# rvignolo/RayTracing.jl

Measured on NVIDIA B200. Metric: segments/sec for segmentize!, higher is better.
Workload: dtype f64

## Files before the change

### raytracing.jl_b200/csrc/eval3.cuh

```cuda
#pragma once
#include "topo.cuh"

namespace rt {

#ifndef RT_EVAL3_THREADS
#define RT_EVAL3_THREADS 32
#endif
constexpr int kEval3Threads = RT_EVAL3_THREADS;
#ifndef RT_EVAL3_MIN_BLOCKS
#define RT_EVAL3_MIN_BLOCKS 32
#endif
#ifndef RT_EVAL3_ALIGN
#define RT_EVAL3_ALIGN 8
#endif
#ifndef RT_EVAL3_PF_AHEAD
#define RT_EVAL3_PF_AHEAD 64
#endif

__device__ __forceinline__ void prefetch_l2(const void *p) { asm volatile("prefetch.global.L2 [%0];" ::"l"(p)); }

__device__ __forceinline__ bool eval3_cross(const Line &trk, const Line &L, P2 &out, bool &redo) {
    const double a = trk.b * L.a, b = L.b * trk.a;
    const double fa = fabs(a), fb = fabs(b);
    const bool par = fabs(a - b) <= kRtol * (fa > fb ? fa : fb);
    const Recip rd = recip_prepare(a - b);
    bool ok = rd.ok;
    out.x = div_try<false>(trk.c * L.b - L.c * trk.b, rd, ok);
    out.y = div_try<false>(trk.a * L.c - L.a * trk.c, rd, ok);
    redo = !ok;
    return par;
}

__global__ void __launch_bounds__(kEval3Threads, RT_EVAL3_MIN_BLOCKS) k_eval3(const __grid_constant__ WalkParams P) {
    const unsigned FULL = 0xffffffffu;
    const DevMesh &m = P.m;
    const int lane = threadIdx.x & 31;
    const long long w = blockIdx.x * (long long)(kEval3Threads / 32) + (threadIdx.x >> 5);
    const long long slot = P.unit_begin + (w >> 5);
    if (slot >= P.unit_end) return;
    if (P.cancel && *P.cancel) return;
    const int ls = (int)(w & 31);
    const long long unit = P.ch.order ? P.ch.order[slot] : slot;
#if RT_EVAL3_PF_AHEAD > 0
    {
        const long long slot_a = slot + RT_EVAL3_PF_AHEAD;
        if (slot_a < P.unit_end) {
            const long long unit_a = P.ch.order ? P.ch.order[slot_a] : slot_a;
            const long long cidx_a = unit_a * 32 + ls;
            const char *recs = (const char *)(P.pool + (cidx_a - P.pool_slot_base) * kRecBlock);
            if (lane < 4) prefetch_l2(recs + 128 * lane);
            else if (lane == 4) prefetch_l2(P.ch.count + cidx_a);
            else if (lane == 5) prefetch_l2(P.ch.prefix + cidx_a);
            else if (lane == 6) prefetch_l2(P.ch.seed_qx + cidx_a);
            else if (lane == 7) prefetch_l2(P.ch.seed_qy + cidx_a);
        }
    }
#endif
    const long long cidx = unit * 32 + ls;
    const int pb0 = (int)(cidx - P.pool_slot_base);
    int pb = pb0;
    const int cnt = P.ch.count[cidx];
    const int rec_first = P.pool[(long long)pb * kRecBlock + lane];
    const int prefix = P.ch.prefix[cidx];
    const double seedx = P.ch.seed_qx[cidx], seedy = P.ch.seed_qy[cidx];
    const int blk = P.ch.unit_block[unit];
    const long long t = 32LL * blk + ls;
    if (t >= P.n_tracks || t < P.trk_begin || t >= P.trk_end) return;
    const int nch = P.ch.nch[t];
    const long long ubase = P.ch.unit_base[blk];
    const int az = P.t.azim[t];
    const Line trk{P.t.a[t], P.t.b[t], P.t.c[t]};
    const long long off_t = P.offsets[t];
    const int j = (int)(unit - ubase);
    if (j >= nch) return;
    if (cnt <= 0) return;
    int rec_cur = lane < cnt ? rec_first : 1;
    int rec_prev = 1;
    int rec;

    const unsigned long long pol_keep = l2_policy_keep();
    const bool right = P.ang.phi[az] < kPi / 2;
    const double delta = P.vol ? P.ang.delta_eff[az] : 0.0;
    const long long base = off_t - P.offset_base + prefix;
    double cqx = seedx, cqy = seedy;
    int cfast = j > 0;
    double lsum = 0.0;
    bool bad = false, any_lit = false;
    const int rot = (lane + 31) & 31;

    const int sh = (int)(base & (RT_EVAL3_ALIGN - 1));
    const int src_lane = (lane - sh) & 31;
    for (int i0 = 0; i0 < cnt + sh; i0 += 32) {
        const int v = i0 + lane - sh;
        int rec_next = 1;
        {
            const int i1 = i0 + 32;
            if (i1 < cnt && (i1 & (kRecBlock - 1)) == 0) pb = P.pool_next[pb];
            if (i1 + lane < cnt) rec_next = P.pool[(long long)pb * kRecBlock + ((i1 + lane) & (kRecBlock - 1))];
        }
        {
            const int a = __shfl_sync(FULL, rec_prev, src_lane), b = __shfl_sync(FULL, rec_cur, src_lane);
            rec = lane < sh ? a : b;
        }
        const bool fast = (rec & 1) == 0;
        const unsigned h = (unsigned)rec >> 2;
        const unsigned cell = fast ? h / 3u : h;
        const unsigned kin = h - 3u * cell;
        const bool exit1 = (rec & 2) != 0;
        P2 q{0.0, 0.0};
        bool par = false, redo = false;
        Line L{0.0, 0.0, 0.0};
        if (fast) {
            unsigned kout = kin + (exit1 ? 1u : 2u);
            kout = kout >= 3u ? kout - 3u : kout;
            double elen;
            ldg256_keep(m.edges + (3u * cell + kout), pol_keep, L.a, L.b, L.c, elen);
            par = eval3_cross(trk, L, q, redo);
        }
        if (redo) par = intersection(trk, L, q);
        const double rx = __shfl_sync(FULL, q.x, rot), ry = __shfl_sync(FULL, q.y, rot);
        const int rfast = __shfl_sync(FULL, (int)fast, rot);
        const bool from_left = lane != 0 && v != 0;
        P2 p{from_left ? rx : cqx, from_left ? ry : cqy};
        const bool have = (from_left ? rfast : cfast) != 0;
        cqx = rx;
        cqy = ry;
        cfast = rfast;
        if (fast && !have) {
            double elen;
            ldg256_keep(m.edges + (3u * cell + kin), pol_keep, L.a, L.b, L.c, elen);
            intersection(trk, L, p);
        }
        if (fast) {
            const double dx = p.x - q.x, dy = p.y - q.y;
            const double l = sqrt(dx * dx + dy * dy);
            const long long so = base + v;
            P.opx[so] = p.x;
            P.opy[so] = p.y;
            P.oqx[so] = q.x;
            P.oqy[so] = q.y;
            P.olen[so] = l;
            P.oelem[so] = (int)cell + 1;
            if (P.vol) atomicAdd(&P.vol[cell], delta * l);
            lsum += l;
            const bool kin_lt_kout = (kin == 0u) || (kin == 1u && exit1);
            const bool lt = right ? (p.x < q.x) : (p.x > q.x);
            const bool in_first = lt || (p.x == q.x && !kin_lt_kout);
            bad = bad || par || !in_first || !(l > P.lmin);
        } else if ((unsigned)v < (unsigned)cnt) {
            any_lit = true;
        }
        rec_prev = rec_cur;
        rec_cur = rec_next;
    }
    if (bad) atomicExch(P.verify_fail, 1);

    if (__any_sync(FULL, any_lit)) {
        pb = pb0;
        for (int i0 = 0; i0 < cnt; i0 += 32) {
            if (i0 && (i0 & (kRecBlock - 1)) == 0) pb = P.pool_next[pb];
            const int v = i0 + lane;
            const int r = v < cnt ? P.pool[(long long)pb * kRecBlock + (v & (kRecBlock - 1))] : 0;
            if (r & 1) {
                const int cell = r >> 2;
                P2 p, q;
                int e_p, e_q;
                intersections(m, cell, trk, right, p, q, e_p, e_q);
                const double l = norm2(p.x - q.x, p.y - q.y);
                const long long so = base + v;
                P.opx[so] = p.x;
                P.opy[so] = p.y;
                P.oqx[so] = q.x;
                P.oqy[so] = q.y;
                P.olen[so] = l;
                P.oelem[so] = cell + 1;
                if (P.vol) atomicAdd(&P.vol[cell], delta * l);
                lsum += l;
            }
        }
    }
    if (P.tsum) {
        for (int o = 16; o > 0; o >>= 1) lsum += __shfl_down_sync(FULL, lsum, o);
        if (lane == 0) atomicAdd(&P.tsum[t], lsum);
    }
}

}
```

### raytracing.jl_b200/csrc/rt_b200.cu

```cuda
#include "../../include/rt_b200.h"

#include <dlfcn.h>

#include <algorithm>
#include <cstdarg>
#include <cstdio>
#include <cstring>
#include <string>
#include <vector>

#include "scan.cuh"
#include "sweep.cuh"
#include "eval3.cuh"
#include "march.cuh"
#include "topo.cuh"
#include "trace.cuh"

using namespace rt;

typedef struct ncclComm *ncclComm_t;
typedef struct {
    char internal[128];
} ncclUniqueId;
typedef int ncclResult_t;
// ... 55 lines not shown
    cudaEvent_t ev_aux = nullptr;
    bool area_valid = false;
    long long *h_pin = nullptr;
    DevBuf b_cell_bin;
    DevBuf b_scratch, b_gcounts, b_gcursor;
    DevBuf b_tsum;
    DevBuf b_pool, b_pool_next, b_pool_cursor;
    int count_batches = 0;
    unsigned long long trace_gen = 0;
    struct PlanKey {
        unsigned long long gen = ~0ULL;
        double chunk_len = -1.0;
        int band = -1, order_grid = -1;
        double band_min = -1.0, band_div = -1.0;
        long long n = -1;
        bool operator==(const PlanKey &o) const { return gen == o.gen && chunk_len == o.chunk_len && band == o.band && order_grid == o.order_grid && n == o.n &&
                   band_min == o.band_min && band_div == o.band_div; }
    } plan_key;
    bool plan_has_order = false;
    int opt_debug_clear_pool = 0;
    double opt_band_cost = 28.0;
    int opt_plan_cache = 1;
    int opt_optimistic = 1;
    bool skip_optimistic_once = false;
    int optimistic_cancels = 0;
    unsigned long long fit_gen = ~0ULL;

    int opt_band_chunks = 1;
    double opt_band_min = 0.0625;
    double opt_band_div = 8.0;
    long long opt_pool_slots = 0;
    double opt_pool_extra = 1.25;
    int opt_pipeline = 3;
    int verify_fallbacks = 0;
    int opt_debug_verify_fail = 0;
    double tau_ms = 0.0;
    cudaEvent_t ev2[2] = {nullptr, nullptr};
    int opt_order_grid = 32;
    const int *order_eval = nullptr;
    int opt_order_classes = 3;
    int n_sm = 148;
    long long n_units = 0;
    double opt_chunk_segments = 208.0;
    double opt_target_walkers = 148.0 * 2048.0 * 4.0;
    double sum_len = 0.0;
    double edge_sum = 0.0, area = 0.0;
    long long total_segments = 0;
    long long cap_cfg = 0;
    long long cap = 0;
    DevBuf b_seg_d, b_seg_e;
    double *s_px = nullptr, *s_py = nullptr, *s_qx = nullptr, *s_qy = nullptr, *s_len = nullptr;
    int *s_elem = nullptr;
    long long res_trk_begin = 0, res_trk_end = 0, res_off_base = 0, res_nseg = 0;
    bool vol_valid = false;

    double phase_ms[6] = {0, 0, 0, 0, 0, 0};
    double stats[8] = {0, 0, 0, 0, 0, 0, 0, 0};

    NcclApi nccl;
    ncclComm_t comm = nullptr;
    int n_ranks = 1, rank = 0;
    cudaStream_t coll_stream = nullptr;
    DevBuf b_vol_alt;
    int vol_cur = 0;
    double *vol_acc = nullptr;
    cudaEvent_t ev_fill_done = nullptr;
    cudaEvent_t ev_vol_free[2] = {nullptr, nullptr};
    bool ev_vol_used[2] = {false, false};
    bool voln_done = false;
    int voln_ready = -1;
};

static inline unsigned long long *d_counters(rt_ctx *c) { return (unsigned long long *)c->b_ctrl.p; }
static inline unsigned long long *d_bad(rt_ctx *c) { return (unsigned long long *)c->b_ctrl.p + 4; }
static inline int *d_verify(rt_ctx *c) { return (int *)((unsigned long long *)c->b_ctrl.p + 5); }
static inline int *d_guard(rt_ctx *c) { return (int *)((unsigned long long *)c->b_ctrl.p + 5) + 1; }
constexpr int kPinWords = 32, kPinCtrlInit = 16, kPinCtrl = 24;

static int fail(rt_ctx *c, int code, const char *fmt, ...) {
    char buf[512];
    va_list ap;
    va_start(ap, fmt);
    vsnprintf(buf, sizeof(buf), fmt, ap);
    va_end(ap);
    if (c) c->err = buf;
    return code;
}

#define CK(call)                                                                                              \
    do {                                                                                                      \
        cudaError_t e_ = (call);                                                                              \
        if (e_ != cudaSuccess)                                                                                \
            return fail(ctx, RT_ERR_CUDA, "%s failed at %s:%d: %s", #call, __FILE__, __LINE__,              \
                        cudaGetErrorString(e_));                                                              \
    } while (0)

static cudaError_t ensure(DevBuf &b, size_t bytes) {
    if (bytes <= b.bytes && b.p) return cudaSuccess;
    if (b.p) cudaFree(b.p);
    b.p = nullptr;
    b.bytes = 0;
    cudaError_t e = cudaMalloc(&b.p, bytes ? bytes : 1);
    if (e == cudaSuccess) b.bytes = bytes;
    return e;
}
static void release(DevBuf &b) {
    if (b.p) cudaFree(b.p);
    b.p = nullptr;
    b.bytes = 0;
}

static inline unsigned blocks_for(long long n, int threads) { return (unsigned)((n + threads - 1) / threads); }

template <typename Tin, typename Tout>
static cudaError_t exclusive_scan(rt_ctx *ctx, const Tin *in, Tout *out, long long n, Tout carry = Tout(0), ScanGuard guard = ScanGuard{}) {
    long long n_tiles = (n + kScanTile - 1) / kScanTile;
    cudaError_t e = ensure(ctx->b_tile, sizeof(Tout) * (size_t)n_tiles);
    if (e != cudaSuccess) return e;
    Tout *tiles = (Tout *)ctx->b_tile.p;
    k_scan_tile_sums<Tin, Tout><<<(unsigned)n_tiles, kScanThreads, 0, ctx->stream>>>(in, tiles, n);
    k_scan_tile_offsets<Tout><<<1, kScanThreads, 0, ctx->stream>>>(tiles, n_tiles);
    k_scan_apply<Tin, Tout><<<(unsigned)n_tiles, kScanThreads, 0, ctx->stream>>>(in, out, tiles, n, carry, guard);
    return cudaGetLastError();
}

extern "C" const char *rt_version(void) { return "rt_b200 0.1 (sm_100a, fp64, fmad=false)"; }

extern "C" int rt_create(rt_ctx **out, int device) {
    if (!out) return RT_ERR_ARG;
    *out = nullptr;
    int n = 0;
    cudaError_t e = cudaGetDeviceCount(&n);
    if (e != cudaSuccess || n <= 0 || device < 0 || device >= n) return RT_ERR_CUDA;
    rt_ctx *ctx = new rt_ctx();
    ctx->device = device;
    cudaDeviceGetAttribute(&ctx->n_sm, cudaDevAttrMultiProcessorCount, device);
    if (ctx->n_sm <= 0) ctx->n_sm = 148;
    if (cudaSetDevice(device) != cudaSuccess || cudaStreamCreateWithFlags(&ctx->stream, cudaStreamNonBlocking) != cudaSuccess ||
        cudaEventCreate(&ctx->tev[0]) != cudaSuccess || cudaEventCreate(&ctx->tev[1]) != cudaSuccess ||
        cudaEventCreate(&ctx->ev2[0]) != cudaSuccess || cudaEventCreate(&ctx->ev2[1]) != cudaSuccess) {
        delete ctx;
        return RT_ERR_CUDA;
    }
    if (cudaHostAlloc((void **)&ctx->h_pin, kPinWords * sizeof(long long), cudaHostAllocDefault) != cudaSuccess) {
        delete ctx;
        return RT_ERR_NOMEM;
    }
    for (int ph = 0; ph < 6; ++ph)
        for (int q = 0; q < 2; ++q)
            if (cudaEventCreate(&ctx->pev[ph][q]) != cudaSuccess) {
                delete ctx;
                return RT_ERR_CUDA;
            }
    *out = ctx;
    return RT_OK;
}

extern "C" void rt_destroy(rt_ctx *ctx) {
    if (!ctx) return;
    cudaSetDevice(ctx->device);
    if (ctx->coll_stream) cudaStreamSynchronize(ctx->coll_stream);
    if (ctx->stream) cudaStreamSynchronize(ctx->stream);
    if (ctx->comm && ctx->nccl.CommDestroy) ctx->nccl.CommDestroy(ctx->comm);
    DevBuf *all[] = {&ctx->b_cell_ptrs, &ctx->b_xy,      &ctx->b_cell_nodes, &ctx->b_nc_ptrs,  &ctx->b_nc_data, &ctx->b_nbr,     &ctx->b_cells,
                     &ctx->b_edges,   &ctx->b_qual,       &ctx->b_bdist,    &ctx->b_sc,      &ctx->b_grid_ptrs, &ctx->b_grid_nodes,
                     &ctx->b_ang_d,   &ctx->b_ang_i,      &ctx->b_trk_d,    &ctx->b_trk_i,   &ctx->b_trk_l,   &ctx->b_trk_c,
                     &ctx->b_err,     &ctx->b_count,      &ctx->b_status,   &ctx->b_offsets, &ctx->b_tile,    &ctx->b_vol,
                     &ctx->b_voln,    &ctx->b_ctrl,       &ctx->b_seg_d,   &ctx->b_seg_e,
                     &ctx->b_twin,    &ctx->b_he,         &ctx->b_node_reach,
                     &ctx->b_nch,     &ctx->b_blk_chunks, &ctx->b_unit_base, &ctx->b_unit_block, &ctx->b_ch_i, &ctx->b_ch_d,
                     &ctx->b_order,   &ctx->b_okeys,      &ctx->b_ohist,     &ctx->b_tsum,
                     &ctx->b_scratch, &ctx->b_gcounts,   &ctx->b_gcursor,   &ctx->b_cell_bin,
                     &ctx->b_omega,   &ctx->b_sigma,     &ctx->b_tau,
                     &ctx->b_pool,    &ctx->b_pool_next, &ctx->b_pool_cursor,
                     &ctx->b_area,    &ctx->b_factor,    &ctx->b_layout,    &ctx->b_vol_alt,  &ctx->b_exc};
    for (DevBuf *b : all) release(*b);
    for (int ph = 0; ph < 6; ++ph)
        for (int q = 0; q < 2; ++q)
            if (ctx->pev[ph][q]) cudaEventDestroy(ctx->pev[ph][q]);
    if (ctx->coll_stream) {
        cudaStreamSynchronize(ctx->coll_stream);
        cudaStreamDestroy(ctx->coll_stream);
    }
    for (cudaEvent_t e : {ctx->ev_fill_done, ctx->ev_vol_free[0], ctx->ev_vol_free[1]})
        if (e) cudaEventDestroy(e);
    if (ctx->aux_stream) cudaStreamDestroy(ctx->aux_stream);
    if (ctx->ev_aux) cudaEventDestroy(ctx->ev_aux);
    if (ctx->stream) cudaStreamDestroy(ctx->stream);
    if (ctx->h_pin) cudaFreeHost(ctx->h_pin);
    delete ctx;
}

extern "C" const char *rt_last_error(const rt_ctx *ctx) { return ctx ? ctx->err.c_str() : "null context"; }

extern "C" int rt_host_alloc(void **ptr, size_t bytes) {
    return cudaHostAlloc(ptr, bytes ? bytes : 1, cudaHostAllocDefault) == cudaSuccess ? RT_OK : RT_ERR_NOMEM;
}
extern "C" int rt_host_free(void *ptr) { return cudaFreeHost(ptr) == cudaSuccess ? RT_OK : RT_ERR_CUDA; }

static void tic(rt_ctx *ctx, int ph) { cudaEventRecord(ctx->pev[ph][0], ctx->stream); }
static void toc(rt_ctx *ctx, int ph) {
    cudaEventRecord(ctx->pev[ph][1], ctx->stream);
    ctx->pev_dirty[ph] = true;
}
static void collect_phase_ms(rt_ctx *ctx) {
    for (int ph = 0; ph < 6; ++ph) {
        if (!ctx->pev_dirty[ph]) continue;
        float ms = 0.f;
        if (cudaEventSynchronize(ctx->pev[ph][1]) == cudaSuccess && cudaEventElapsedTime(&ms, ctx->pev[ph][0], ctx->pev[ph][1]) == cudaSuccess)
            ctx->phase_ms[ph] = (double)ms;
        ctx->pev_dirty[ph] = false;
    }
}

extern "C" int rt_mesh_upload(rt_ctx *ctx, int32_t n_nodes, const double *xy, int32_t n_cells, const int32_t *cell_ptrs,
                              const int32_t *cell_data, const int32_t *node_cell_ptrs, const int32_t *node_cell_data,
                              const double bb_min[2], const double bb_max[2]) {
    if (!ctx) return RT_ERR_ARG;
    if (n_nodes < 3 || n_cells < 1 || !xy || !cell_ptrs || !cell_data || (!node_cell_ptrs != !node_cell_data) || (!bb_min != !bb_max))
        return fail(ctx, RT_ERR_ARG, "rt_mesh_upload: null or empty mesh arrays");
    const bool dev_nc = node_cell_ptrs == nullptr;
    const bool dev_bb = bb_min == nullptr;
    bool mixed = false;
    for (int32_t c = 0; c < n_cells; ++c) {
        const int nn = cell_ptrs[c + 1] - cell_ptrs[c];
        if (nn == 4)
            mixed = true;
        else if (nn != 3)
            return fail(ctx, RT_ERR_ARG, "rt_mesh_upload: cell %d has %d nodes (triangles and quadrilaterals only)", c + 1, nn);
    }
    if (mixed && dev_nc) return fail(ctx, RT_ERR_ARG, "rt_mesh_upload: a mesh with quadrilaterals needs the vertex -> cells table from the caller");
    const size_t n_cd = (size_t)(cell_ptrs[n_cells] - 1);
    CK(cudaSetDevice(ctx->device));
    cudaStream_t st = ctx->stream;
    tic(ctx, 0);
    size_t n_nc = dev_nc ? (size_t)3 * n_cells : (size_t)(node_cell_ptrs[n_nodes] - 1);
    CK(ensure(ctx->b_xy, sizeof(double2) * (size_t)n_nodes));
    CK(ensure(ctx->b_cell_nodes, sizeof(int) * n_cd));
    CK(ensure(ctx->b_nc_ptrs, sizeof(int) * ((size_t)n_nodes + 1)));
    CK(ensure(ctx->b_nc_data, sizeof(int) * n_nc));
    CK(ensure(ctx->b_nbr, sizeof(int) * 3 * (size_t)n_cells));
    CK(ensure(ctx->b_cells, sizeof(CellRec) * (size_t)n_cells));
    CK(ensure(ctx->b_edges, sizeof(EdgeRec) * 3 * (size_t)n_cells));
    CK(ensure(ctx->b_qual, sizeof(float) * (size_t)n_cells));
    CK(ensure(ctx->b_bdist, sizeof(float) * (size_t)n_cells));
    CK(ensure(ctx->b_sc, sizeof(MeshScalars)));
    const size_t tab_n[3] = {n_cd, dev_nc ? 0 : (size_t)n_nodes + 1, dev_nc ? 0 : n_nc};
    CK(ensure(ctx->b_scratch, sizeof(int32_t) * (tab_n[0] + tab_n[1] + tab_n[2])));
    CK(cudaMemcpyAsync(ctx->b_xy.p, xy, sizeof(double) * 2 * (size_t)n_nodes, cudaMemcpyHostToDevice, st));
    const int32_t *tab_src[3] = {cell_data, node_cell_ptrs, node_cell_data};
    void *tab_dst[3] = {ctx->b_cell_nodes.p, ctx->b_nc_ptrs.p, ctx->b_nc_data.p};
    size_t tab_off = 0;
    for (int q = 0; q < 3; ++q) {
        if (tab_n[q] == 0) continue;
        int32_t *stage = (int32_t *)ctx->b_scratch.p + tab_off;
        CK(cudaMemcpyAsync(stage, tab_src[q], sizeof(int32_t) * tab_n[q], cudaMemcpyHostToDevice, st));
        k_to_zero_based<<<blocks_for((long long)tab_n[q], 256), 256, 0, st>>>(stage, (int *)tab_dst[q], (long long)tab_n[q]);
        tab_off += tab_n[q];
    }

    if (mixed) {
        DevBuf stage;
        CK(ensure(stage, sizeof(int32_t) * ((size_t)n_cells + 1)));
        CK(ensure(ctx->b_cell_ptrs, sizeof(int) * ((size_t)n_cells + 1)));
        CK(cudaMemcpyAsync(stage.p, cell_ptrs, sizeof(int32_t) * ((size_t)n_cells + 1), cudaMemcpyHostToDevice, st));
        k_to_zero_based<<<blocks_for((long long)n_cells + 1, 256), 256, 0, st>>>((const int32_t *)stage.p, (int *)ctx->b_cell_ptrs.p, (long long)n_cells + 1);
        CK(cudaStreamSynchronize(st));
        release(stage);
    }
    if (dev_nc) {
        DevBuf deg, cur;
        CK(ensure(deg, sizeof(int) * (size_t)n_nodes));
        CK(ensure(cur, sizeof(int) * (size_t)n_nodes));
        CK(cudaMemsetAsync(deg.p, 0, sizeof(int) * (size_t)n_nodes, st));
        CK(cudaMemsetAsync(cur.p, 0, sizeof(int) * (size_t)n_nodes, st));
        k_nc_count<<<blocks_for(3LL * n_cells, 256), 256, 0, st>>>(n_cells, (const int *)ctx->b_cell_nodes.p, (int *)deg.p);
        CK((exclusive_scan<int, int>(ctx, (const int *)deg.p, (int *)ctx->b_nc_ptrs.p, (long long)n_nodes)));
        k_nc_fill<<<blocks_for(3LL * n_cells, 256), 256, 0, st>>>(n_cells, (const int *)ctx->b_cell_nodes.p, (const int *)ctx->b_nc_ptrs.p,
                                                                   (int *)cur.p, (int *)ctx->b_nc_data.p);
        k_nc_sort<<<blocks_for(n_nodes, 256), 256, 0, st>>>(n_nodes, (const int *)ctx->b_nc_ptrs.p, (int *)ctx->b_nc_data.p);
        CK(cudaGetLastError());
        CK(cudaStreamSynchronize(st));
        release(deg);
        release(cur);
    }
    double bbv[4];
    if (dev_bb) {
        DevBuf dbb;
        CK(ensure(dbb, sizeof(double) * 4));
        const double init[4] = {INFINITY, INFINITY, -INFINITY, -INFINITY};
        CK(cudaMemcpyAsync(dbb.p, init, sizeof(init), cudaMemcpyHostToDevice, st));
        k_bbox<<<std::min(1024u, blocks_for(n_nodes, 256)), 256, 0, st>>>((const double2 *)ctx->b_xy.p, n_nodes, (double *)dbb.p);
        CK(cudaMemcpyAsync(bbv, dbb.p, sizeof(bbv), cudaMemcpyDeviceToHost, st));
        CK(cudaStreamSynchronize(st));
        release(dbb);
        bb_min = bbv;
        bb_max = bbv + 2;
    }
    DevMesh &m = ctx->m;
    m.n_nodes = n_nodes;
    m.n_cells = n_cells;
    m.xy = (const double2 *)ctx->b_xy.p;
    m.cell_nodes = (const int *)ctx->b_cell_nodes.p;
    m.cell_ptrs = mixed ? (const int *)ctx->b_cell_ptrs.p : nullptr;
    m.nc_ptrs = (const int *)ctx->b_nc_ptrs.p;
    m.nc_data = (const int *)ctx->b_nc_data.p;
// ... 1304 lines not shown
    if (r != 0) return fail(ctx, RT_ERR_NCCL, "ncclCommInitRank: %s", ctx->nccl.GetErrorString ? ctx->nccl.GetErrorString(r) : "?");
    if (!ctx->coll_stream) {
        if (cudaStreamCreateWithFlags(&ctx->coll_stream, cudaStreamNonBlocking) != cudaSuccess ||
            cudaEventCreateWithFlags(&ctx->ev_fill_done, cudaEventDisableTiming) != cudaSuccess ||
            cudaEventCreateWithFlags(&ctx->ev_vol_free[0], cudaEventDisableTiming) != cudaSuccess ||
            cudaEventCreateWithFlags(&ctx->ev_vol_free[1], cudaEventDisableTiming) != cudaSuccess)
            return fail(ctx, RT_ERR_CUDA, "rt_comm_init: cannot create the collective stream");
    }
    ctx->n_ranks = n_ranks;
    ctx->rank = rank;
    return RT_OK;
}

extern "C" int rt_volumes(rt_ctx *ctx, double *volumes) {
    if (!ctx) return RT_ERR_ARG;
    const bool have = ctx->segmented && ctx->vol_valid;
    const bool coll = ctx->comm && ctx->coll_stream;
    if (!have && !(coll && ctx->has_mesh)) return fail(ctx, RT_ERR_ARG, "rt_volumes: run rt_segmentize with volumes enabled first");
    CK(cudaSetDevice(ctx->device));
    cudaStream_t st = ctx->stream;
    int nc = ctx->m.n_cells;
    CK(ensure(ctx->b_voln, sizeof(double) * ((size_t)nc + 1)));
    const double *src = ctx->vol_acc ? ctx->vol_acc : (const double *)ctx->b_vol.p;
    if (!have) {
        CK(cudaStreamSynchronize(ctx->coll_stream));
        CK(ensure(ctx->b_vol, sizeof(double) * ((size_t)nc + 1)));
        CK(cudaMemsetAsync(ctx->b_vol.p, 0, sizeof(double) * ((size_t)nc + 1), st));
        const double one = 1.0;
        CK(cudaMemcpyAsync((double *)ctx->b_vol.p + nc, &one, sizeof(double), cudaMemcpyHostToDevice, st));
        CK(cudaStreamSynchronize(st));
        src = (const double *)ctx->b_vol.p;
    }
    if (coll) {
        cudaStream_t cs = ctx->coll_stream;
        CK(cudaEventRecord(ctx->ev_fill_done, st));
        CK(cudaStreamWaitEvent(cs, ctx->ev_fill_done, 0));
        CK(cudaEventRecord(ctx->pev[5][0], cs));
        ncclResult_t r = ctx->nccl.AllReduce(src, ctx->b_voln.p, (size_t)nc + 1, ncclFloat64, ncclSum, ctx->comm, cs);
        if (r != 0) return fail(ctx, RT_ERR_NCCL, "ncclAllReduce: %s", ctx->nccl.GetErrorString ? ctx->nccl.GetErrorString(r) : "?");
        k_normalise<<<blocks_for(nc, 256), 256, 0, cs>>>((const double *)ctx->b_voln.p, (double *)ctx->b_voln.p, nc, (double)ctx->n2);
        CK(cudaGetLastError());
        CK(cudaEventRecord(ctx->pev[5][1], cs));
        ctx->pev_dirty[5] = true;
        if (have) {
            CK(cudaEventRecord(ctx->ev_vol_free[ctx->vol_cur], cs));
            ctx->ev_vol_used[ctx->vol_cur] = true;
            ctx->voln_ready = ctx->vol_cur;
        }
        if (volumes || !have) CK(cudaStreamSynchronize(cs));
        if (!have) return fail(ctx, RT_ERR_ARG, "rt_volumes: this rank's rt_segmentize failed; it joined the all-reduce with a zero contribution and the failed-rank flag");
    } else {
        if (!ctx->voln_done) {
            tic(ctx, 5);
            k_normalise<<<blocks_for(nc, 256), 256, 0, st>>>(src, (double *)ctx->b_voln.p, nc, (double)ctx->n2);
            CK(cudaGetLastError());
            toc(ctx, 5);
        }
        ctx->voln_ready = -1;
        if (volumes) CK(cudaStreamSynchronize(st));
    }
    if (volumes) {
        CK(cudaMemcpy(volumes, ctx->b_voln.p, sizeof(double) * (size_t)nc, cudaMemcpyDeviceToHost));
        if (coll) {
            double failed = 0.0;
            CK(cudaMemcpy(&failed, (const double *)ctx->b_voln.p + nc, sizeof(double), cudaMemcpyDeviceToHost));
            if (failed != 0.0)
                return fail(ctx, RT_ERR_PEER, "rt_volumes: rt_segmentize failed on %d rank(s) of the communicator: the volumes miss their tracks", (int)failed);
        }
    }
    return RT_OK;
}


__device__ __forceinline__ unsigned long long splitmix64(unsigned long long &x) {
    unsigned long long z = (x += 0x9e3779b97f4a7c15ull);
    z = (z ^ (z >> 30)) * 0xbf58476d1ce4e5b9ull;
    z = (z ^ (z >> 27)) * 0x94d049bb133111ebull;
    return z ^ (z >> 31);
}

__global__ void k_selftest_division(long long n, unsigned long long seed, int exp_span, unsigned long long *mismatch) {
    long long i = blockIdx.x * (long long)blockDim.x + threadIdx.x;
    if (i >= n) return;
    unsigned long long st = seed + 0x632be59bd9b4e019ull * (unsigned long long)(i + 1);
    unsigned long long bad = 0;
    for (int rep = 0; rep < 64; ++rep) {
        unsigned long long r1 = splitmix64(st), r2 = splitmix64(st), r3 = splitmix64(st);
        int e1 = 1023 + (int)(r3 % (2 * exp_span + 1)) - exp_span, e2 = 1023 + (int)((r3 >> 20) % (2 * exp_span + 1)) - exp_span;
        e1 = min(max(e1, 0), 2046);
        e2 = min(max(e2, 1), 2046);
        unsigned long long mx = r1 & 0xfffffffffffffull, mn = r2 & 0xfffffffffffffull;
        int kind = (int)((r3 >> 44) & 15);
        if (kind == 1) mx = 0;
        if (kind == 2) mx = 0xfffffffffffffull;
        if (kind == 3) mn = 0xfffffffffffffull;
        if (kind == 4) mn = 0;
        double x = __longlong_as_double((long long)(((r1 >> 63) << 63) | ((unsigned long long)e1 << 52) | mx));
        double d = __longlong_as_double((long long)(((r2 >> 63) << 63) | ((unsigned long long)e2 << 52) | mn));
        if (kind == 5) x = 0.0;
        if (kind == 6) x = -0.0;
        Recip r = recip_prepare(d);
        double q1 = div_shared(x, r), q2 = x / d;
        if (__double_as_longlong(q1) != __double_as_longlong(q2)) bad++;
    }
    if (bad) atomicAdd(mismatch, bad);
}

extern "C" int rt_selftest_division(rt_ctx *ctx, int64_t n_threads, uint64_t seed, int32_t exp_span, int64_t *mismatches) {
    if (!ctx || !mismatches || n_threads < 1 || exp_span < 0 || exp_span > 1022) return RT_ERR_ARG;
    CK(cudaSetDevice(ctx->device));
    DevBuf d;
    CK(ensure(d, sizeof(unsigned long long)));
    CK(cudaMemsetAsync(d.p, 0, sizeof(unsigned long long), ctx->stream));
    k_selftest_division<<<blocks_for(n_threads, 256), 256, 0, ctx->stream>>>(n_threads, seed, exp_span, (unsigned long long *)d.p);
    CK(cudaGetLastError());
    unsigned long long h = 0;
    CK(cudaMemcpyAsync(&h, d.p, sizeof(h), cudaMemcpyDeviceToHost, ctx->stream));
    CK(cudaStreamSynchronize(ctx->stream));
    release(d);
    *mismatches = (int64_t)h;
    return RT_OK;
}

extern "C" int rt_stats(rt_ctx *ctx, double stats[8]) {
    if (!ctx || !stats) return RT_ERR_ARG;
    cudaSetDevice(ctx->device);
    collect_phase_ms(ctx);
    ctx->stats[5] = ctx->phase_ms[2];
    ctx->stats[6] = ctx->phase_ms[4];
    ctx->stats[7] = ctx->phase_ms[3];
    memcpy(stats, ctx->stats, sizeof(ctx->stats));
    return RT_OK;
}

extern "C" int rt_info(rt_ctx *ctx, const char *key, double *value) {
    if (!ctx || !key || !value) return RT_ERR_ARG;
    std::string k(key);
    if (k == "verify_fallbacks")
        *value = ctx->verify_fallbacks;
    else if (k == "tau_ms")
        *value = ctx->tau_ms;
    else if (k == "n_units")
        *value = (double)ctx->n_units;
    else if (k == "segment_capacity")
        *value = (double)ctx->cap;
    else if (k == "rho")
        *value = ctx->area > 0.0 ? ctx->edge_sum / (kPi * ctx->area) : 0.0;
    else if (k == "band_cost")
        *value = ctx->opt_band_cost;
    else if (k == "count_batches")
        *value = (double)ctx->count_batches;
    else if (k == "optimistic_cancels")
        *value = (double)ctx->optimistic_cancels;
    else
        return fail(ctx, RT_ERR_ARG, "rt_info: unknown key %s", key);
    return RT_OK;
}

extern "C" int rt_debug_chunk_stats(rt_ctx *ctx, double out[8]) {
    if (!ctx || !out || !ctx->segmented || ctx->n_units <= 0) return fail(ctx, RT_ERR_ARG, "rt_debug_chunk_stats: call rt_segmentize first");
    CK(cudaSetDevice(ctx->device));
    CK(cudaStreamSynchronize(ctx->stream));
    const long long n = ctx->n_shard, n_units = ctx->n_units, n_blocks = (n + 31) / 32;
    const size_t nc = (size_t)n_units * 32;
    std::vector<int> nch((size_t)n), ublk((size_t)n_units), seed(nc), cnt(nc);
    std::vector<long long> ubase((size_t)n_blocks + 1);
    CK(cudaMemcpy(nch.data(), ctx->b_nch.p, sizeof(int) * nch.size(), cudaMemcpyDeviceToHost));
    CK(cudaMemcpy(ublk.data(), ctx->b_unit_block.p, sizeof(int) * ublk.size(), cudaMemcpyDeviceToHost));
    CK(cudaMemcpy(ubase.data(), ctx->b_unit_base.p, sizeof(long long) * ubase.size(), cudaMemcpyDeviceToHost));
    CK(cudaMemcpy(seed.data(), ctx->b_ch_i.p, sizeof(int) * nc, cudaMemcpyDeviceToHost));
    CK(cudaMemcpy(cnt.data(), (const int *)ctx->b_ch_i.p + 2 * nc, sizeof(int) * nc, cudaMemcpyDeviceToHost));
    double work = 0, voids = 0, sum = 0, mx = 0;
    for (long long u = 0; u < n_units; ++u) {
        const long long b = ublk[(size_t)u];
        const int j = (int)(u - ubase[(size_t)b]);
        for (int l = 0; l < 32; ++l) {
            const long long t = 32 * b + l;
            if (t >= n || j >= nch[(size_t)t]) continue;
            const size_t c = (size_t)u * 32 + l;
            if (j >= 1 && seed[c] < 0) voids += 1;
            if (cnt[c] > 0) {
                work += 1;
                sum += cnt[c];
                mx = std::max(mx, (double)cnt[c]);
            }
        }
    }
    const double mean = work > 0 ? sum / work : 0.0;
    double over15 = 0, over2 = 0;
    for (long long u = 0; u < n_units; ++u) {
        const long long b = ublk[(size_t)u];
        const int j = (int)(u - ubase[(size_t)b]);
        double umax = 0, usum = 0;
        for (int l = 0; l < 32; ++l) {
            const long long t = 32 * b + l;
            if (t >= n || j >= nch[(size_t)t]) continue;
            const double c = (double)std::max(cnt[(size_t)u * 32 + l], 0);
            umax = std::max(umax, c);
            usum += c;
        }
        over15 += umax;
        over2 += usum / 32.0;
    }
    out[0] = work;
    out[1] = voids;
    out[2] = mean;
    out[3] = mx;
    out[4] = over15;
    out[5] = over2;
    out[6] = (double)nc;
    out[7] = (double)n_units;
    return RT_OK;
}

extern "C" int rt_phase_ms(rt_ctx *ctx, double ms[6]) {
    if (!ctx || !ms) return RT_ERR_ARG;
    cudaSetDevice(ctx->device);
    collect_phase_ms(ctx);
    memcpy(ms, ctx->phase_ms, sizeof(ctx->phase_ms));
    return RT_OK;
}

extern "C" int rt_timer_start(rt_ctx *ctx) {
    if (!ctx) return RT_ERR_ARG;
    CK(cudaSetDevice(ctx->device));
    if (ctx->coll_stream) CK(cudaStreamSynchronize(ctx->coll_stream));
    CK(cudaStreamSynchronize(ctx->stream));
    CK(cudaEventRecord(ctx->tev[0], ctx->stream));
    return RT_OK;
}

extern "C" int rt_timer_stop(rt_ctx *ctx, double *elapsed_ms) {
    if (!ctx || !elapsed_ms) return RT_ERR_ARG;
    if (ctx->voln_ready >= 0) CK(cudaStreamWaitEvent(ctx->stream, ctx->ev_vol_free[ctx->voln_ready], 0));
    CK(cudaEventRecord(ctx->tev[1], ctx->stream));
    CK(cudaEventSynchronize(ctx->tev[1]));
    float ms = 0.f;
    CK(cudaEventElapsedTime(&ms, ctx->tev[0], ctx->tev[1]));
    *elapsed_ms = (double)ms;
    return RT_OK;
}

extern "C" int rt_set_option(rt_ctx *ctx, const char *name, double value) {
    if (!ctx || !name) return RT_ERR_ARG;
    std::string n(name);
    if (n == "chunk_segments" && value >= 1.0)
        ctx->opt_chunk_segments = value;
    else if (n == "target_walkers" && value >= 1.0)
        ctx->opt_target_walkers = value;
    else if (n == "order_grid" && value >= 0.0 && value <= 256.0)
        ctx->opt_order_grid = (int)value;
    else if (n == "pipeline" && (value == 0.0 || value == 1.0 || value == 3.0))
        ctx->opt_pipeline = (int)value;
    else if (n == "debug_clear_pool")
        ctx->opt_debug_clear_pool = value != 0.0;
    else if (n == "band_cost" && value >= 0.0)
        ctx->opt_band_cost = value;
    else if (n == "order_classes" && value >= 0.0 && value <= 64.0)
        ctx->opt_order_classes = (int)value;
    else if (n == "plan_cache")
        ctx->opt_plan_cache = value != 0.0;
    else if (n == "optimistic")
        ctx->opt_optimistic = value != 0.0;
    else if (n == "band_chunks")
        ctx->opt_band_chunks = value != 0.0;
    else if (n == "band_min" && value >= 0.0)
        ctx->opt_band_min = value;
    else if (n == "band_div" && value >= 1.0 && value <= 64.0)
        ctx->opt_band_div = value;
    else if (n == "pool_slots" && value >= 0.0)
        ctx->opt_pool_slots = (long long)value;
    else if (n == "pool_extra" && value >= 0.0)
        ctx->opt_pool_extra = value;
    else if (n == "debug_verify_fail")
        ctx->opt_debug_verify_fail = value != 0.0;
    else
        return fail(ctx, RT_ERR_ARG, "rt_set_option: unknown option or bad value: %s", name);
    return RT_OK;
}
```

Measured before the change: 32.91 billion.

## Stage segment outputs in shared-memory ring and flush with bulk async copies

Replaces the per-lane scattered global stores of segment columns with writes into a per-warp shared-memory ring. Full windows are then flushed to global memory by TMA bulk copies (cp.async.bulk) issued by lane 0, and unaligned edge elements are stored directly. This removes the old alignment-shift shuffle path and aims to produce fully coalesced, asynchronous output writes. In exchange it adds about 6KB of shared memory per one-warp block, which may cut occupancy, and adds proxy fences and wait_group synchronisation.

```diff
diff --git a/raytracing.jl_b200/csrc/eval3.cuh b/raytracing.jl_b200/csrc/eval3.cuh
--- a/raytracing.jl_b200/csrc/eval3.cuh
+++ b/raytracing.jl_b200/csrc/eval3.cuh
@@ -10,14 +10,34 @@
 #ifndef RT_EVAL3_MIN_BLOCKS
 #define RT_EVAL3_MIN_BLOCKS 32
 #endif
-#ifndef RT_EVAL3_ALIGN
-#define RT_EVAL3_ALIGN 8
-#endif
+#ifndef RT_EVAL3_WIN
+#define RT_EVAL3_WIN 64
+#endif
+#ifndef RT_EVAL3_FLUSH
+#define RT_EVAL3_FLUSH 1
+#endif
+constexpr int kEval3Win = RT_EVAL3_WIN;
+constexpr int kEval3Ring = 2 * kEval3Win;
 #ifndef RT_EVAL3_PF_AHEAD
 #define RT_EVAL3_PF_AHEAD 64
 #endif
 
 __device__ __forceinline__ void prefetch_l2(const void *p) { asm volatile("prefetch.global.L2 [%0];" ::"l"(p)); }
+
+__device__ __forceinline__ void bulk_s2g(void *dst, const void *src, int bytes) {
+    asm volatile("cp.async.bulk.global.shared::cta.bulk_group [%0], [%1], %2;" ::"l"(dst), "r"((unsigned)__cvta_generic_to_shared(src)),
+                 "r"(bytes)
+                 : "memory");
+}
+__device__ __forceinline__ void bulk_commit() { asm volatile("cp.async.bulk.commit_group;" ::: "memory"); }
+template <int N>
+__device__ __forceinline__ void bulk_wait_read() {
+    asm volatile("cp.async.bulk.wait_group.read %0;" ::"n"(N) : "memory");
+}
+__device__ __forceinline__ void stg_f64x2(double *p, double2 v) { asm volatile("st.global.v2.f64 [%0], {%1,%2};" ::"l"(p), "d"(v.x), "d"(v.y) : "memory"); }
+__device__ __forceinline__ void stg_s32x4(int *p, int4 v) {
+    asm volatile("st.global.v4.s32 [%0], {%1,%2,%3,%4};" ::"l"(p), "r"(v.x), "r"(v.y), "r"(v.z), "r"(v.w) : "memory");
+}
 
 __device__ __forceinline__ bool eval3_cross(const Line &trk, const Line &L, P2 &out, bool &redo) {
     const double a = trk.b * L.a, b = L.b * trk.a;
@@ -75,8 +95,6 @@
     if (j >= nch) return;
     if (cnt <= 0) return;
     int rec_cur = lane < cnt ? rec_first : 1;
-    int rec_prev = 1;
-    int rec;
 
     const unsigned long long pol_keep = l2_policy_keep();
     const bool right = P.ang.phi[az] < kPi / 2;
@@ -88,20 +106,48 @@
     bool bad = false, any_lit = false;
     const int rot = (lane + 31) & 31;
 
-    const int sh = (int)(base & (RT_EVAL3_ALIGN - 1));
-    const int src_lane = (lane - sh) & 31;
-    for (int i0 = 0; i0 < cnt + sh; i0 += 32) {
-        const int v = i0 + lane - sh;
+    static_assert(kEval3Threads == 32, "the staging ring belongs to the block: one warp per block");
+    __shared__ __align__(16) double s_d[5][kEval3Ring];
+    __shared__ __align__(16) int s_e[kEval3Ring];
+    double *const col[5] = {P.opx, P.opy, P.oqx, P.oqy, P.olen};
+    const int bs = (int)(base & (kEval3Ring - 1));
+    const long long base0 = base - bs;
+    const int d_lo = (bs + 1) & ~1, d_hi = (bs + cnt) & ~1, e_lo = (bs + 3) & ~3, e_hi = (bs + cnt) & ~3;
+    int fu = bs;
+    auto flush = [&](int f, int h) {
+        const int d0 = max(f, d_lo), d1 = min(h, d_hi), e0 = max(f, e_lo), e1 = min(h, e_hi);
+#if RT_EVAL3_FLUSH == 1
+        if (lane == 0) {
+            if (d1 > d0)
+                for (int c = 0; c < 5; ++c) bulk_s2g(col[c] + base0 + d0, &s_d[c][d0 & (kEval3Ring - 1)], 8 * (d1 - d0));
+            if (e1 > e0) bulk_s2g(P.oelem + base0 + e0, &s_e[e0 & (kEval3Ring - 1)], 4 * (e1 - e0));
+            bulk_commit();
+        }
+#else
+        static_assert(kEval3Win <= 64, "one 16-byte store per lane and column");
+        const int k = d0 + 2 * lane, s = k & (kEval3Ring - 1);
+        if (k < d1) {
+            const long long o = base0 + k;
+            stg_f64x2(P.opx + o, *(const double2 *)&s_d[0][s]);
+            stg_f64x2(P.opy + o, *(const double2 *)&s_d[1][s]);
+            stg_f64x2(P.oqx + o, *(const double2 *)&s_d[2][s]);
+            stg_f64x2(P.oqy + o, *(const double2 *)&s_d[3][s]);
+            stg_f64x2(P.olen + o, *(const double2 *)&s_d[4][s]);
+        }
+        const int ke = e0 + 4 * lane;
+        if (ke < e1) stg_s32x4(P.oelem + base0 + ke, *(const int4 *)&s_e[ke & (kEval3Ring - 1)]);
+#endif
+    };
+
+    for (int i0 = 0; i0 < cnt; i0 += 32) {
+        const int v = i0 + lane;
         int rec_next = 1;
         {
             const int i1 = i0 + 32;
             if (i1 < cnt && (i1 & (kRecBlock - 1)) == 0) pb = P.pool_next[pb];
             if (i1 + lane < cnt) rec_next = P.pool[(long long)pb * kRecBlock + ((i1 + lane) & (kRecBlock - 1))];
         }
-        {
-            const int a = __shfl_sync(FULL, rec_prev, src_lane), b = __shfl_sync(FULL, rec_cur, src_lane);
-            rec = lane < sh ? a : b;
-        }
+        const int rec = rec_cur;
         const bool fast = (rec & 1) == 0;
         const unsigned h = (unsigned)rec >> 2;
         const unsigned cell = fast ? h / 3u : h;
@@ -120,7 +166,7 @@
         if (redo) par = intersection(trk, L, q);
         const double rx = __shfl_sync(FULL, q.x, rot), ry = __shfl_sync(FULL, q.y, rot);
         const int rfast = __shfl_sync(FULL, (int)fast, rot);
-        const bool from_left = lane != 0 && v != 0;
+        const bool from_left = lane != 0;
         P2 p{from_left ? rx : cqx, from_left ? ry : cqy};
         const bool have = (from_left ? rfast : cfast) != 0;
         cqx = rx;
@@ -131,31 +177,68 @@
             ldg256_keep(m.edges + (3u * cell + kin), pol_keep, L.a, L.b, L.c, elen);
             intersection(trk, L, p);
         }
+        const int a = bs + i0;
+#if RT_EVAL3_FLUSH == 1
+        if (lane == 0) {
+            if (a / kEval3Win != (a + 31) / kEval3Win) bulk_wait_read<0>();
+            else bulk_wait_read<1>();
+        }
+#endif
+        __syncwarp();
         if (fast) {
             const double dx = p.x - q.x, dy = p.y - q.y;
             const double l = sqrt(dx * dx + dy * dy);
-            const long long so = base + v;
-            P.opx[so] = p.x;
-            P.opy[so] = p.y;
-            P.oqx[so] = q.x;
-            P.oqy[so] = q.y;
-            P.olen[so] = l;
-            P.oelem[so] = (int)cell + 1;
+            const int u = bs + v, s = u & (kEval3Ring - 1);
+            s_d[0][s] = p.x;
+            s_d[1][s] = p.y;
+            s_d[2][s] = q.x;
+            s_d[3][s] = q.y;
+            s_d[4][s] = l;
+            s_e[s] = (int)cell + 1;
+            if (u < d_lo || u >= d_hi) {
+                const long long so = base + v;
+                P.opx[so] = p.x;
+                P.opy[so] = p.y;
+                P.oqx[so] = q.x;
+                P.oqy[so] = q.y;
+                P.olen[so] = l;
+            }
+            if (u < e_lo || u >= e_hi) P.oelem[base + v] = (int)cell + 1;
             if (P.vol) atomicAdd(&P.vol[cell], delta * l);
             lsum += l;
             const bool kin_lt_kout = (kin == 0u) || (kin == 1u && exit1);
             const bool lt = right ? (p.x < q.x) : (p.x > q.x);
             const bool in_first = lt || (p.x == q.x && !kin_lt_kout);
             bad = bad || par || !in_first || !(l > P.lmin);
-        } else if ((unsigned)v < (unsigned)cnt) {
+        } else if (v < cnt) {
             any_lit = true;
         }
-        rec_prev = rec_cur;
+        const int e_it = bs + min(i0 + 32, cnt);
+        const bool last = i0 + 32 >= cnt;
+#if RT_EVAL3_FLUSH == 1
+        if (last || (fu / kEval3Win + 1) * kEval3Win <= e_it)
+            asm volatile("fence.proxy.async.shared::cta;" ::: "memory");
+#endif
+        __syncwarp();
+        while (fu < e_it) {
+            const int wend = (fu / kEval3Win + 1) * kEval3Win;
+            if (wend > e_it && !last) break;
+            const int hu = min(wend, e_it);
+            flush(fu, hu);
+            fu = hu;
+        }
         rec_cur = rec_next;
     }
     if (bad) atomicExch(P.verify_fail, 1);
 
     if (__any_sync(FULL, any_lit)) {
+#if RT_EVAL3_FLUSH == 1
+        if (lane == 0) asm volatile("cp.async.bulk.wait_group 0;" ::: "memory");
+        __syncwarp();
+        asm volatile("fence.proxy.async.global;" ::: "memory");
+#else
+        __syncwarp();
+#endif
         pb = pb0;
         for (int i0 = 0; i0 < cnt; i0 += 32) {
             if (i0 && (i0 & (kRecBlock - 1)) == 0) pb = P.pool_next[pb];
@@ -179,6 +262,9 @@
             }
         }
     }
+#if RT_EVAL3_FLUSH == 1
+    if (lane == 0) bulk_wait_read<0>();
+#endif
     if (P.tsum) {
         for (int o = 16; o > 0; o >>= 1) lsum += __shfl_down_sync(FULL, lsum, o);
         if (lane == 0) atomicAdd(&P.tsum[t], lsum);
diff --git a/raytracing.jl_b200/csrc/rt_b200.cu b/raytracing.jl_b200/csrc/rt_b200.cu
--- a/raytracing.jl_b200/csrc/rt_b200.cu
+++ b/raytracing.jl_b200/csrc/rt_b200.cu
@@ -231,6 +231,10 @@
                 delete ctx;
                 return RT_ERR_CUDA;
             }
+    if (cudaFuncSetAttribute(k_eval3, cudaFuncAttributePreferredSharedMemoryCarveout, cudaSharedmemCarveoutMaxShared) != cudaSuccess) {
+        delete ctx;
+        return RT_ERR_CUDA;
+    }
     *out = ctx;
     return RT_OK;
 }
@@ -1841,6 +1845,12 @@
         *value = (double)ctx->count_batches;
     else if (k == "optimistic_cancels")
         *value = (double)ctx->optimistic_cancels;
+    else if (k == "eval3_blocks_per_sm") {
+        int nb = 0;
+        CK(cudaSetDevice(ctx->device));
+        CK(cudaOccupancyMaxActiveBlocksPerMultiprocessor(&nb, k_eval3, kEval3Threads, 0));
+        *value = nb;
+    }
     else
         return fail(ctx, RT_ERR_ARG, "rt_info: unknown key %s", key);
     return RT_OK;
```

New measurement: 29.07 billion (median of 6 runs). 0.883x the previous value.
